# CIS565-Fall-2017/Project3-CUDA-Path-Tracer

Hardware: AMD Instinct MI355X
Metric: Mrays/sec (live paths x bounces) at 800x800 Cornell depth 8 (higher is better)
Workload: dtype f32

## Files before the change

### project3-cuda-path-tracer_amd/csrc/pt_device.hpp

```cpp
#pragma once
#include <hip/hip_runtime.h>
#include <stdint.h>

namespace ptd {

struct f3 { float x, y, z; };

#define PTD __device__ __forceinline__

PTD f3 mk(float x, float y, float z) { f3 r; r.x = x; r.y = y; r.z = z; return r; }
PTD f3 add(f3 a, f3 b) { return mk(a.x + b.x, a.y + b.y, a.z + b.z); }
PTD f3 sub(f3 a, f3 b) { return mk(a.x - b.x, a.y - b.y, a.z - b.z); }
PTD f3 mul(f3 a, f3 b) { return mk(a.x * b.x, a.y * b.y, a.z * b.z); }
PTD f3 scale(f3 a, float s) { return mk(a.x * s, a.y * s, a.z * s); }
PTD f3 neg(f3 a) { return mk(-a.x, -a.y, -a.z); }
PTD float dot(f3 a, f3 b) { return (a.x * b.x + a.y * b.y) + a.z * b.z; }
PTD float length_gated(f3 a);
PTD f3 normalize_gated(f3 a);
PTD float sqrt_gated(float x);
PTD float length(f3 a) { return length_gated(a); }
PTD f3 normalize(f3 a) { return normalize_gated(a); }
PTD f3 normalize_unit(f3 a);
PTD f3 cross(f3 x, f3 y) {
    return mk(x.y * y.z - y.y * x.z, x.z * y.x - y.z * x.x, x.x * y.y - y.x * x.y);
}
PTD f3 cross_axis(f3 x, f3 y) {
    return mk(__builtin_fmaf(x.y, y.z, -(y.y * x.z)), __builtin_fmaf(x.z, y.x, -(y.z * x.x)), __builtin_fmaf(x.x, y.y, -(y.x * x.y)));
}
PTD f3 reflect(f3 I, f3 N) {
    const f3 p = scale(N, dot(N, I));
    return mk(__builtin_fmaf(-2.0f, p.x, I.x), __builtin_fmaf(-2.0f, p.y, I.y), __builtin_fmaf(-2.0f, p.z, I.z));
}

PTD uint32_t utilhash(uint32_t a) {
    a = (a + 0x7ed55d16u) + (a << 12);
    a = (a ^ 0xc761c23cu) ^ (a >> 19);
    a = (a + 0x165667b1u) + (a << 5);
    a = (a + 0xd3a2646cu) ^ (a << 9);
    a = (a + 0xfd7046c5u) + (a << 3);
    a = (a ^ 0xb55a4f09u) ^ (a >> 16);
    return a;
}

PTD uint32_t mod_m31(uint64_t x) {
    uint32_t r = (uint32_t)(x & 0x7fffffffull) + (uint32_t)(x >> 31);
    return r >= 0x7fffffffu ? r - 0x7fffffffu : r;
}

PTD uint32_t lcg_seed(uint32_t s) {
    uint32_t r = mod_m31((uint64_t)s);
    return r == 0u ? 1u : r;
}

PTD uint32_t seeded_engine(int iter, int index, int depth) {
    uint32_t k = (1u << 31) | ((uint32_t)depth << 22) | (uint32_t)iter;
    return lcg_seed(utilhash(k) ^ utilhash((uint32_t)index));
}

PTD float u01(uint32_t &state) {
    state = mod_m31(48271ull * (uint64_t)state);
    return (float)(state - 1u) / 2147483648.0f;
}

PTD void sincos_shared(float x, float &s, float &c) {
    const float TWO_OVER_PI = 0.636619772367581343f;
    const float MAGIC = 12582912.0f;
    const float P1 = 1.57079625129699707031f, P2 = 7.54978941586159635335e-08f, P3 = 5.39030285815811905290e-15f;
    const float S1 = -1.66666671633720398e-01f, S2 = 8.33333190530538559e-03f,
                S3 = -1.98401714442297816e-04f, S4 = 2.72681563728838228e-06f;
    const float C1 = 4.16666530072689056e-02f, C2 = -1.38876168057322502e-03f, C3 = 2.44678121816832572e-05f;
    const float kf = __builtin_fmaf(x, TWO_OVER_PI, MAGIC) - MAGIC;
    const float r1 = __builtin_fmaf(-kf, P1, x);
    const float r = __builtin_fmaf(-kf, P2, r1);
    const float rl = __builtin_fmaf(-kf, P3, __builtin_fmaf(-kf, P2, r1 - r));
    const float z = r * r;
    const float ze = __builtin_fmaf(r, r, -z);
    const float ps = __builtin_fmaf(z, __builtin_fmaf(z, __builtin_fmaf(z, S4, S3), S2), S1);
    const float pc = __builtin_fmaf(z, __builtin_fmaf(z, C3, C2), C1);
    const float hz = 0.5f * z;
    const float w = 1.0f - hz;
    float e = (1.0f - w) - hz;
    e = __builtin_fmaf(-0.5f, ze, e);
    const float u = (r * z) * ps;
    const float sn = r + __builtin_fmaf(rl, w, u);
    const float cs = w + __builtin_fmaf(z * z, pc, __builtin_fmaf(-rl, sn, e));
    const int q = (int)kf & 3;
    float so = (q & 1) ? cs : sn;
    float co = (q & 1) ? sn : cs;
    so = (q & 2) ? -so : so;
    co = ((q + 1) & 2) ? -co : co;
    s = so;
    c = co;
}

PTD f3 hemisphere(f3 normal, uint32_t &rng) {
    const float TWO_PI = 6.2831853071795864769252867665590057683943f;
    const float SQRT_OF_ONE_THIRD = 0.5773502691896257645091487805019574556476f;
    float up = sqrt_gated(u01(rng));
    float over = sqrt_gated(1 - up * up);
    float around = u01(rng) * TWO_PI;
    f3 notN;
    if (__builtin_fabsf(normal.x) < SQRT_OF_ONE_THIRD) notN = mk(1, 0, 0);
    else if (__builtin_fabsf(normal.y) < SQRT_OF_ONE_THIRD) notN = mk(0, 1, 0);
    else notN = mk(0, 0, 1);
    f3 p1 = normalize(cross_axis(normal, notN));
    f3 p2 = normalize_unit(cross(normal, p1));
    float sa, ca;
    sincos_shared(around, sa, ca);
    return add(add(scale(normal, up), scale(p1, ca * over)), scale(p2, sa * over));
}

constexpr int GEOM_WORDS = 40;
constexpr int G_INV = 4, G_FWD = 16, G_INVT = 28;
constexpr int MAT_WORDS = 12;

template <typename P> PTD f3 mv_point(P m, f3 v) {
    f3 r;
    r.x = (m[0] * v.x + m[3] * v.y) + (m[6] * v.z + m[9]);
    r.y = (m[1] * v.x + m[4] * v.y) + (m[7] * v.z + m[10]);
    r.z = (m[2] * v.x + m[5] * v.y) + (m[8] * v.z + m[11]);
    return r;
}
template <typename P> PTD f3 mv_dir(P m, f3 v) {
    f3 r;
    r.x = (m[0] * v.x + m[3] * v.y) + __builtin_fmaf(m[9], 0.0f, m[6] * v.z);
    r.y = (m[1] * v.x + m[4] * v.y) + __builtin_fmaf(m[10], 0.0f, m[7] * v.z);
    r.z = (m[2] * v.x + m[5] * v.y) + __builtin_fmaf(m[11], 0.0f, m[8] * v.z);
    return r;
}

PTD f3 point_on_ray(f3 o, f3 d, float t) { return add(o, scale(normalize_unit(d), (t - .0001f))); }

struct Hit {
    float t;
    int geom;
    int outside;
    f3 aux;
};

PTD f3 face_from_code(int code) {
    const float s = (code & 1) ? 1.0f : -1.0f;
    const int axis = code >> 1;
    return mk(axis == 0 ? s : 0.0f, axis == 1 ? s : 0.0f, axis == 2 ? s : 0.0f);
}

#ifndef PT_FASTDIV
#define PT_FASTDIV 1
#endif
PTD float rcp_refined(float d) {
    float r = __builtin_amdgcn_rcpf(d);
    float e = __builtin_fmaf(-d, r, 1.0f);
    return __builtin_fmaf(e, r, r);
}
PTD float div_by_rcp(float n, float d, float r) {
    float q = n * r;
    float e = __builtin_fmaf(-d, q, n);
    q = __builtin_fmaf(e, r, q);
    e = __builtin_fmaf(-d, q, n);
    return __builtin_fmaf(e, r, q);
}
PTD void sqrt_newton(float x, float &s, float &h) {
    const float y = __builtin_amdgcn_rsqf(x);
    float g = x * y;
    h = 0.5f * y;
    const float r = __builtin_fmaf(-h, g, 0.5f);
    g = __builtin_fmaf(g, r, g);
    h = __builtin_fmaf(h, r, h);
    s = __builtin_fmaf(__builtin_fmaf(-g, g, x), h, g);
}
PTD float sqrt_normal_range(float x) {
    float s, h;
    sqrt_newton(x, s, h);
    return s;
}
PTD float rsqrt_of_root(float x) {
    float s, h;
    sqrt_newton(x, s, h);
    float q = __uint_as_float(__float_as_uint(h + h) + 1u);
    q = __builtin_fmaf(__builtin_fmaf(-s, q, 1.0f), q, q);
    return __builtin_fmaf(__builtin_fmaf(-s, q, 1.0f), q, q);
}
constexpr float NEAR_ONE_LO = 0x1.ffep-1f, NEAR_ONE_HI = 0x1.001p+0f;
PTD float rsqrt_near_one(float x) {
    const float e = x - 1.0f;
    const float w = __builtin_fmaf(e, -0.5f, 0x1.8p-25f);
    const float t = w + (1.0f + 0x1p-10f);
    return t - 0x1p-10f;
}
#ifndef PT_WAVE_ALL_BALLOT
#define PT_WAVE_ALL_BALLOT 1
#endif
PTD bool wave_all(bool p) {
#if PT_WAVE_ALL_BALLOT
    return __builtin_amdgcn_ballot_w64(!p) == 0ull;
#else
    return __all(p);
#endif
}
PTD bool in_range_bits(float x, float lo, float hi) {
    return (__float_as_uint(x) - __float_as_uint(lo)) <= (__float_as_uint(hi) - __float_as_uint(lo));
}
PTD bool all_in_range(float x, float lo, float hi) {
#if PT_FASTDIV
    return wave_all(in_range_bits(x, lo, hi));
#else
    (void)x; (void)lo; (void)hi;
    return false;
#endif
}
// ... 227 lines not shown
```

### project3-cuda-path-tracer_amd/csrc/pt_h_scene.hpp

```cpp
#pragma once

namespace {

int upload_tri_bounds(const pt_scene_desc *d, double Rorigin);

int upload_cull(const pt_scene_desc *d, const pt_camera &cam) {
    const int n = d->num_geoms;
    std::vector<const float *> inv((size_t)std::max(1, n));
    std::vector<char> sph((size_t)std::max(1, n)), skip((size_t)std::max(1, n));
    for (int i = 0; i < n; ++i) {
        inv[(size_t)i] = &d->geoms[i].inverseTransform.m[0][0];
        sph[(size_t)i] = d->geoms[i].type == PT_SPHERE;
        skip[(size_t)i] = d->geoms[i].type == PT_TRIANGLE_MESH;
    }
    const double eye[3] = {(double)cam.position.x, (double)cam.position.y, (double)cam.position.z};
    std::vector<ptcull::Box> boxes;
    std::vector<double> pts(eye, eye + 3);
    for (int t = 0; t < d->num_triangles; ++t) {
        const pt_vec3 *v = &d->triangles[t].v0;
        double m = 0.0;
        for (int k = 0; k < 3; ++k) m = std::max(m, (double)std::fabs(v[k].x) + std::fabs(v[k].y) + std::fabs(v[k].z));
        if (t == 0 || m > pts[3]) { if (pts.size() < 6) pts.resize(6, 0.0); pts[3] = m; pts[4] = 0.0; pts[5] = 0.0; }
    }
    R.scene.rmax = ptcull::make_boxes(inv.data(), reinterpret_cast<const bool *>(sph.data()),
                                      reinterpret_cast<const bool *>(skip.data()), n, pts.data(), (int)(pts.size() / 3), boxes);
    std::vector<float> rec((size_t)std::max(1, n) * CULL_WORDS, 0.0f);
    for (int i = 0; i < n; ++i) {
        float *r = rec.data() + (size_t)i * CULL_WORDS;
        for (int k = 0; k < 3; ++k) ptcull::centre_half(boxes[(size_t)i].lo[k], boxes[(size_t)i].hi[k], r[2 * k], r[2 * k + 1]);
        int ax = 3;
        if (d->geoms[i].type == PT_CUBE && !pt_experiment("PTMI355_NO_AXIS_REJECT"))
            ax = ptcull::reject_row(&d->geoms[i].inverseTransform.m[0][0], &r[7]);
        if (ax == 4 && pt_experiment("PTMI355_NO_ROW_REJECT")) ax = 3;
        const int tw = d->geoms[i].type | (ax << 8);
        memcpy(&r[6], &tw, 4);
        const uint32_t ent = ((uint32_t)d->geoms[i].type << 7) | ((uint32_t)i << 9);
        memcpy(&r[11], &ent, 4);
    }
    if (!R.d_cull) HIPCHK(hipMalloc(&R.d_cull, rec.size() * 4));
    HIPCHK(hipMemcpyAsync(R.d_cull, rec.data(), rec.size() * 4, hipMemcpyHostToDevice, R.stream));
    HIPCHK(hipStreamSynchronize(R.stream));
    R.scene.cull = R.d_cull;
    R.cull_eye_reach = std::fabs(eye[0]) + std::fabs(eye[1]) + std::fabs(eye[2]);
    return upload_tri_bounds(d, (double)R.scene.rmax);
}

void make_tri_bounds(const pt_triangle *tris, int count, double Rorigin, float *out) {
    const double u = 0x1p-24;
    const float pad = ptbvh::spec_pad(reinterpret_cast<const float *>(tris), count);
    const int n4 = (count + 3) & ~3;
    for (int i = 0; i < n4; ++i) {
        float *o = out + (size_t)i * 4;
        if (i >= count) { o[0] = o[1] = o[2] = 0.0f; o[3] = -1.0f; continue; }
        const pt_triangle &t = tris[i];
        const float v0[3] = {t.v0.x, t.v0.y, t.v0.z};
        const float e1[3] = {t.v1.x - t.v0.x, t.v1.y - t.v0.y, t.v1.z - t.v0.z};
        const float e2[3] = {t.v2.x - t.v0.x, t.v2.y - t.v0.y, t.v2.z - t.v0.z};
        double c[3], h2 = 0.0, cinf = 0.0;
        bool fin = true;
        for (int a = 0; a < 3; ++a) {
            const float x1 = v0[a] + e1[a], x2 = v0[a] + e2[a];
            const float lo = std::fmin(v0[a], std::fmin(x1, x2)) - pad, hi = std::fmax(v0[a], std::fmax(x1, x2)) + pad;
            if (!std::isfinite(lo) || !std::isfinite(hi)) fin = false;
            c[a] = 0.5 * ((double)lo + (double)hi);
            const double h = 0.5 * ((double)hi - (double)lo);
            h2 += h * h;
            cinf = std::fmax(cinf, std::fabs(c[a]));
        }
        if (!fin || !std::isfinite(Rorigin)) { o[0] = o[1] = o[2] = 0.0f; o[3] = INFINITY; continue; }
        const double R0 = std::sqrt(h2);
        const double reach = Rorigin + cinf + R0;
        const double delta = 2.0 * 1.7320508075688772 * u * reach;
        const double Rs = (R0 + 4.0 * (delta + 0x1p-19 * reach)) * (1.0 + 0x1p-10);
        for (int a = 0; a < 3; ++a) o[a] = (float)c[a];
        o[3] = ptcull::round_up(Rs * Rs);
        if (!std::isfinite(o[3])) o[3] = INFINITY;
    }
}

void make_tri_records(const float *spheres, int n, _Float16 *records, float frame[4]) {
    double lo[3] = {INFINITY, INFINITY, INFINITY}, hi[3] = {-INFINITY, -INFINITY, -INFINITY};
    for (int i = 0; i < n; ++i) {
        const float *sp = spheres + (size_t)i * 4;
        if (!(sp[3] >= 0.0f) || !std::isfinite(sp[3])) continue;
        for (int a = 0; a < 3; ++a) { lo[a] = std::fmin(lo[a], (double)sp[a]); hi[a] = std::fmax(hi[a], (double)sp[a]); }
    }
    double g[3] = {0.0, 0.0, 0.0}, Rm = 0.0;
    if (lo[0] <= hi[0]) for (int a = 0; a < 3; ++a) g[a] = (double)(float)(0.5 * (lo[a] + hi[a]));
    for (int i = 0; i < n; ++i) {
        const float *sp = spheres + (size_t)i * 4;
        if (!(sp[3] >= 0.0f) || !std::isfinite(sp[3])) continue;
        const double dx = sp[0] - g[0], dy = sp[1] - g[1], dz = sp[2] - g[2];
        Rm = std::fmax(Rm, std::sqrt(dx * dx + dy * dy + dz * dz) + std::sqrt((double)sp[3]));
    }
    Rm = Rm > 0.0 ? Rm * (1.0 + 0x1p-20) : 1.0;
    float ir = (float)(1.0 / Rm);
    if (!(ir > 0.0f) || !std::isfinite(ir)) ir = 1.0f;
    frame[0] = (float)g[0]; frame[1] = (float)g[1]; frame[2] = (float)g[2]; frame[3] = ir;
    auto pair = [](double v, _Float16 &h, _Float16 &l) { h = (_Float16)(float)v; l = (_Float16)(float)(v - (double)(float)h); };
    for (int i = 0; i < n; ++i) {
        const float *sp = spheres + (size_t)i * 4;
        _Float16 *a = records + (size_t)i * 32;
        for (int k = 0; k < 32; ++k) a[k] = (_Float16)0.0f;
        a[29] = (_Float16)1.0f; a[30] = (_Float16)1.0f;
        if (!(sp[3] >= 0.0f)) { a[27] = (_Float16)30000.0f; continue; }
        if (!std::isfinite(sp[3])) { a[27] = (_Float16)-30000.0f; continue; }
        const double c[3] = {(sp[0] - g[0]) * (double)ir, (sp[1] - g[1]) * (double)ir, (sp[2] - g[2]) * (double)ir};
        const double v[9] = {-c[0] * c[0], -c[1] * c[1], -c[2] * c[2], -2.0 * c[0] * c[1], -2.0 * c[0] * c[2], -2.0 * c[1] * c[2], c[0], c[1], c[2]};
        for (int t = 0; t < 9; ++t) { _Float16 h, l; pair(v[t], h, l); a[3 * t] = h; a[3 * t + 1] = h; a[3 * t + 2] = l; }
        _Float16 h, l;
        pair((c[0] * c[0] + c[1] * c[1] + c[2] * c[2]) - (double)sp[3] * (double)ir * (double)ir, h, l);
        a[27] = h; a[28] = l;
    }
}

int upload_tri_bounds(const pt_scene_desc *d, double Rorigin) {
    if (R.mesh_mode != MESH_TILES || d->num_meshes <= 0) return PT_OK;
    size_t recs = 0;
    for (int k = 0; k < d->num_meshes; ++k) recs += (size_t)((d->meshes[k].triangle_count + 63) & ~63);
    std::vector<_Float16> tr(std::max<size_t>(recs, 64) * 32, (_Float16)0.0f);
    std::vector<float> sph;
    size_t off = 0;
    for (int k = 0; k < d->num_meshes; ++k) {
        const pt_mesh &m = d->meshes[k];
        const size_t n64 = (size_t)((m.triangle_count + 63) & ~63);
        sph.assign(n64 * 4, 0.0f);
        make_tri_bounds(d->triangles + m.first_triangle, m.triangle_count, Rorigin, sph.data());
        for (size_t i = (size_t)((m.triangle_count + 3) & ~3); i < n64; ++i) sph[i * 4 + 3] = -1.0f;
        float frame[4];
        make_tri_records(sph.data(), (int)n64, tr.data() + off * 32, frame);
        float *r = R.grec_frames.data() + (size_t)m.geom_index * 4;
        for (int a = 0; a < 4; ++a) r[a] = frame[a];
        off += n64;
    }
    if (!R.d_tri_bound || R.tri_bound_words < tr.size() / 2) {
        if (R.d_tri_bound) { HIPCHK(hipStreamSynchronize(R.stream)); (void)hipFree(R.d_tri_bound); R.d_tri_bound = nullptr; }
        HIPCHK(hipMalloc(&R.d_tri_bound, tr.size() * 2));
        R.tri_bound_words = tr.size() / 2;
    }
    HIPCHK(hipMemcpyAsync(R.d_tri_bound, tr.data(), tr.size() * 2, hipMemcpyHostToDevice, R.stream));
    for (int k = 0; k < d->num_meshes; ++k) {
        const int gi = d->meshes[k].geom_index;
        HIPCHK(hipMemcpyAsync(R.d_geoms + (size_t)gi * ptd::GEOM_WORDS + ptd::G_INV + 7, R.grec_frames.data() + (size_t)gi * 4, 16, hipMemcpyHostToDevice, R.stream));
    }
    HIPCHK(hipStreamSynchronize(R.stream));
    R.scene.tri_rec = R.d_tri_bound;
    return PT_OK;
}

}

namespace one {

static int upload_bvh(const pt_scene_desc *d, std::vector<float> &grec) {
    std::vector<float> nodes, btris, tops;
    std::vector<int32_t> mesh_list;
    float prune = 0.0f;
    int guard = 1;
    R.bvh_info = pt_bvh_info{};
    R.mesh_grids.clear();
    std::vector<int> by_geom((size_t)d->num_meshes);
    for (int k = 0; k < d->num_meshes; ++k) by_geom[(size_t)k] = k;
    std::sort(by_geom.begin(), by_geom.end(), [&](int x, int y) { return d->meshes[x].geom_index < d->meshes[y].geom_index; });
    for (int kk = 0; kk < d->num_meshes; ++kk) {
        const int k = by_geom[(size_t)kk];
        const pt_mesh &m = d->meshes[k];
        if (kk > 0 && d->meshes[by_geom[(size_t)kk - 1]].geom_index == m.geom_index)
            return fail(PT_ERR_INVALID, "pt_init: geom %d owns more than one mesh", m.geom_index);
        ptbvh::Tree tree;
        ptbvh::build(reinterpret_cast<const float *>(d->triangles + m.first_triangle), m.triangle_count, tree, (double)R.scene.rmax);
        const int root = (int)(nodes.size() / BVH_NODE_WORDS);
        const int slot0 = (int)(btris.size() / TRI_WORDS);
        if ((int64_t)slot0 + m.triangle_count >= (1 << ptbvh::LINK_BITS) || tree.num_nodes() >= (1 << ptbvh::LINK_BITS))
            return fail(PT_ERR_INVALID, "pt_init: PT_MESH_BVH holds at most 2^24 triangles (record links are 24 bits)");
        for (int n = 0; n < tree.num_nodes(); ++n) {
            float *w = &tree.nodes[(size_t)n * BVH_NODE_WORDS];
            for (int c = 0; c < 2; ++c) {
                uint32_t link;
                memcpy(&link, &w[6 + c], 4);
                if ((link >> ptbvh::LINK_BITS) & ptbvh::INFO_LEAF) { link += (uint32_t)slot0; memcpy(&w[6 + c], &link, 4); }
            }
        }
        nodes.insert(nodes.end(), tree.nodes.begin(), tree.nodes.end());
        for (int s = 0; s < m.triangle_count; ++s) {
            const int32_t orig = m.first_triangle + tree.order[(size_t)s];
            const pt_triangle &t = d->triangles[orig];
            float r[TRI_WORDS] = {t.v0.x, t.v0.y, t.v0.z,
                                  t.v1.x - t.v0.x, t.v1.y - t.v0.y, t.v1.z - t.v0.z,
                                  t.v2.x - t.v0.x, t.v2.y - t.v0.y, t.v2.z - t.v0.z, 0.0f, 0.0f, 0.0f};
            memcpy(&r[9], &orig, 4);
// ... 108 lines not shown
```

### project3-cuda-path-tracer_amd/csrc/pt_k_bounce.hpp

```cpp
#pragma once

namespace {

enum { MODE_FUSED = 0, MODE_ISECT = 1, MODE_CACHE0 = 2 };

template <typename T>
__device__ __forceinline__ T karg_field(size_t offset) {
    const __attribute__((address_space(4))) char *kp = (const __attribute__((address_space(4))) char *)__builtin_amdgcn_kernarg_segment_ptr();
    asm volatile("" : "+s"(kp));
    return *(const __attribute__((address_space(4))) T *)(kp + offset);
}
template <typename T>
__device__ __forceinline__ T karg_struct(size_t offset) {
    static_assert(sizeof(T) % 4 == 0, "whole dwords");
    const __attribute__((address_space(4))) char *kp = (const __attribute__((address_space(4))) char *)__builtin_amdgcn_kernarg_segment_ptr();
    asm volatile("" : "+s"(kp));
    uint32_t w[sizeof(T) / 4];
#pragma unroll
    for (size_t k = 0; k < sizeof(T) / 4; ++k) w[k] = *(const __attribute__((address_space(4))) uint32_t *)(kp + offset + 4 * k);
    T t;
    __builtin_memcpy(&t, w, sizeof(T));
    return t;
}
__device__ __forceinline__ Pool karg_pool(size_t offset) {
    return Pool{karg_field<float *>(offset + offsetof(Pool, base)), karg_field<uint32_t>(offset + offsetof(Pool, cap))};
}

struct TileCtx {
    bool kargs = false;
    bool kmisc = false;
    bool epi_direct = false;
    SceneAcc acc;
    float *tri_lds;
    int lane, iter0;
    uint32_t stamp;
};

struct TileRegs {
    bool have, active;
    uint32_t i, src, tile, pid, smp;
    int pixel;
    f3 col;
    MeshBest mb;
};

template <bool GEN, bool RESOLVE = false>
__device__ __forceinline__ void tile_load(const BounceArgs &a, const TileCtx &c, const Pool &in, int depth,
                                          uint32_t tile, uint32_t i, uint32_t src, bool have, bool active,
                                          TileRegs &tr, f3 &ro, f3 &rd) {
    constexpr bool gen_rays = GEN;
    tr.have = have; tr.i = i; tr.src = src; tr.tile = tile;
    tr.pid = DEAD_PID; tr.smp = 0; tr.pixel = 0;
    tr.col = ptd::mk(1.0f, 1.0f, 1.0f);
    tr.mb.t = FLT_MAX; tr.mb.geom = -1; tr.mb.tri = -1;
    ro = ptd::mk(0, 0, 0); rd = ptd::mk(0, 0, 1);
    if (active) {
        if (gen_rays) {
            tr.pid = i;
        } else {
            const SlotPtr p = (c.kargs ? karg_pool(offsetof(BounceArgs, in)) : in).slot(src);
            tr.pid = ppid(p);
            ro = ptd::mk(pf(p, 0), pf(p, 1), pf(p, 2));
            rd = ptd::mk(pf(p, 3), pf(p, 4), pf(p, 5));
            tr.col = ptd::mk(pf(p, 6), pf(p, 7), pf(p, 8));
            if (tr.pid == DEAD_PID) active = false;
        }
    }
    bool pending = false;
    if (RESOLVE && active) { pending = (tr.pid & PENDING_DIR) != 0u; tr.pid &= ~PENDING_DIR; }
    if (active) {
        if (c.kmisc) {
            const TileMap map = karg_struct<TileMap>(offsetof(BounceArgs, map));
            tr.smp = sample_of(map, tr.pid);
            tr.pixel = local_to_pixel(map, (int)(tr.pid - tr.smp * (uint32_t)map.tile_pixels));
            if (gen_rays) camera_ray(karg_struct<pt_camera>(offsetof(BounceArgs, cam)), karg_struct<Lens>(offsetof(BounceArgs, lens)),
                                     karg_field<int>(offsetof(BounceArgs, trace_depth)), c.iter0 + (int)tr.smp, tr.pixel, map.W, ro, rd);
        } else {
            tr.smp = sample_of(a.map, tr.pid);
            tr.pixel = local_to_pixel(a.map, (int)(tr.pid - tr.smp * (uint32_t)a.map.tile_pixels));
            if (gen_rays) camera_ray(a.cam, a.lens, a.trace_depth, c.iter0 + (int)tr.smp, tr.pixel, a.map.W, ro, rd);
        }
    }
    if (RESOLVE && pending) {
        uint32_t rng = ptd::seeded_engine(c.iter0 + (int)tr.smp, tr.pixel, depth - 1);
        rd = ptd::hemisphere(rd, rng);
    }
    tr.active = active;
}

__device__ __forceinline__ bool mesh_root_candidate(const int4 *bvh_meshes, int bvh_nmesh, const float *geoms, const float *bvh_nodes, f3 ro, f3 rd) {
    bool cand = false;
#pragma unroll 1
    for (int k = 0; k < bvh_nmesh; ++k) {
        const __attribute__((address_space(4))) int *mrec =
            (const __attribute__((address_space(4))) int *)(unsigned long long)(bvh_meshes + k);
        cfloat *grid = as_const(geoms) + (size_t)mrec[0] * ptd::GEOM_WORDS + ptd::G_INV;
        const __attribute__((address_space(4))) uint32_t *b =
            (const __attribute__((address_space(4))) uint32_t *)(unsigned long long)(bvh_nodes + (size_t)mrec[1] * BVH_NODE_WORDS);
        const BvhRay br = bvh_ray(ro, rd, ptd::mk(grid[0], grid[1], grid[2]), ptd::mk(grid[3], grid[4], grid[5]));
        float tn, tf;
        bvh_slab(br, b[0], b[1], b[2], tn, tf);
        cand |= tn <= tf;
        bvh_slab(br, b[3], b[4], b[5], tn, tf);
        cand |= tn <= tf;
    }
    return cand;
}
__device__ __forceinline__ bool mesh_root_candidate(const SceneDev &sc, f3 ro, f3 rd) {
    return mesh_root_candidate(sc.bvh_meshes, sc.bvh_nmesh, sc.geoms, sc.bvh_nodes, ro, rd);
}

template <bool COMPACT, int MESH = MESH_NONE, bool SORT = false, bool DEFER = false>
__device__ __forceinline__ void tile_shade(const BounceArgs &a, const TileCtx &c, const Pool &in, const Pool &out, int depth,
                                           const TileRegs &tr, f3 ro, f3 rd, float t, f3 nrm, int mat, int outside,
                                           uint32_t n, uint32_t dst_base, uint32_t &packed, uint32_t &traced,
                                           uint32_t key_stride = 0) {
    const int lane = c.lane;
    bool alive = false, deferred = false;
    ptd::PathState ps;
    ps.o = ro; ps.d = rd; ps.c = tr.col;
    if (tr.active) {
        const bool defer = DEFER && (c.kargs ? karg_field<int>(offsetof(BounceArgs, defer_dir)) : a.defer_dir) != 0;
        alive = ptd::shade_scatter(ps, t, nrm, mat, outside, c.acc.mats, c.iter0 + (int)tr.smp, tr.pixel, depth,
                                   depth == a.trace_depth - 1, defer, &deferred);
        if (!alive) {
            if (c.epi_direct) {
                if (!(ps.c.x == 0.0f && ps.c.y == 0.0f && ps.c.z == 0.0f)) {
                    float *img = karg_field<float *>(offsetof(BounceArgs, epi_image)) + 3 * (size_t)tr.pixel;
                    const float r = img[0] + ps.c.x, g = img[1] + ps.c.y, b = img[2] + ps.c.z;
                    img[0] = r; img[1] = g; img[2] = b;
                    float *host = karg_field<float *>(offsetof(BounceArgs, epi_host));
                    if (host) { host += 3 * (size_t)tr.pixel; host[0] = r; host[1] = g; host[2] = b; }
                }
            } else {
                put_final((c.kargs || c.kmisc) ? karg_field<float *>(offsetof(BounceArgs, fin)) : a.fin, tr.pid, ps.c, c.stamp);
            }
        }
    }
    const uint64_t bal = ballot64(alive);
    const uint64_t act = ballot64(tr.active);
    traced += (uint32_t)__popcll((unsigned long long)act);
    uint32_t dst = tr.i;
    if (COMPACT && SORT) {
        for_each_key(alive, (uint32_t)mat, [&](uint32_t k, uint64_t m) {
            const uint32_t have = (uint32_t)__builtin_amdgcn_readlane((int)packed, (int)k);
            if (alive && (uint32_t)mat == k) dst = k * key_stride + dst_base + have + rank_below(m);
            if ((uint32_t)lane == k) packed += (uint32_t)__popcll((unsigned long long)m);
        });
    } else if (COMPACT) {
        dst = dst_base + packed + rank_below(bal);
        packed += (uint32_t)__popcll((unsigned long long)bal);
    }
    if (alive) {
        const SlotPtr p = (c.kargs ? karg_pool(offsetof(BounceArgs, out)) : out).slot(dst);
        pf(p, 0) = ps.o.x; pf(p, 1) = ps.o.y; pf(p, 2) = ps.o.z;
        pf(p, 3) = ps.d.x; pf(p, 4) = ps.d.y; pf(p, 5) = ps.d.z;
        pf(p, 6) = ps.c.x; pf(p, 7) = ps.c.y; pf(p, 8) = ps.c.z;
        ppid(p) = deferred ? (tr.pid | PENDING_DIR) : tr.pid;
        if (MESH == MESH_PRE) {
            constexpr size_t SC = offsetof(BounceArgs, scene);
            const bool reach = c.kargs
                ? mesh_root_candidate(karg_field<const int4 *>(SC + offsetof(SceneDev, bvh_meshes)), karg_field<int>(SC + offsetof(SceneDev, bvh_nmesh)),
                                      karg_field<const float *>(SC + offsetof(SceneDev, geoms)), karg_field<const float *>(SC + offsetof(SceneDev, bvh_nodes)), ps.o, ps.d)
                : mesh_root_candidate(a.scene, ps.o, ps.d);
            if (reach)
                atomicOr(&(c.kargs ? karg_field<unsigned long long *>(offsetof(BounceArgs, mesh_flags_out)) : a.mesh_flags_out)[dst >> 6], 1ull << (dst & 63u));
        }
    } else if (!COMPACT && tr.have && tr.i < n) {
        out.pid(dst) = DEAD_PID;
    }
}

template <bool COMPACT, int MESH, bool SORT = false, bool DEFER = false>
__device__ __forceinline__ void tile_finish(const BounceArgs &a, const TileCtx &c, const WaveQ &q, int par, const Pool &in,
                                            const Pool &out, int depth, const TileRegs &tr, uint32_t n, uint32_t dst_base,
                                            uint32_t &packed, uint32_t &traced, uint32_t key_stride = 0) {
    const float *ry = q.rays(par) + c.lane;
    const f3 ro = ptd::mk(ry[0], ry[64], ry[128]);
    const f3 rd = ptd::mk(ry[192], ry[256], ry[320]);
    float t = -1.0f; f3 nrm = ptd::mk(0, 0, 0); int mat = 0, outside = 1;
    if (tr.active) tile_result(q, par, c.acc, a.scene.tris, tr.mb, t, nrm, mat, outside);
    tile_shade<COMPACT, MESH, SORT, DEFER>(a, c, in, out, depth, tr, ro, rd, t, nrm, mat, outside, n, dst_base, packed, traced, key_stride);
}

struct WgSpans {
    uint32_t p1, p2, p3, total;
    uint32_t b0, b1, b2, b3;
};

template <int MODE, bool COMPACT, int MESH, bool GEN, bool SORT = false, bool DEFER = false, bool RESOLVE = false>
__device__ __forceinline__ void run_tiles(const BounceArgs &a, const TileCtx &c, WaveQ &q, const Pool &in, const Pool &out,
                                          int depth, uint32_t first_tile, uint32_t count, uint32_t tiles,
                                          uint32_t n, bool packed_in, uint32_t span_in, uint32_t &cur, uint32_t dst_base,
                                          bool own_span, const WgSpans &ws, uint32_t &packed, uint32_t &traced,
                                          uint32_t key_stride = 0, bool aligned = false) {
    const int lane = c.lane;
    bool pending = false;
    TileRegs prev{};
    uint32_t prev_ticket = 0;
    int par = 0;
    const bool masked = MODE == MODE_FUSED && GEN && a.cull0 != nullptr;
    uint32_t mtile = masked ? first_tile % a.cull0_tiles : 0u;
    for (uint32_t r = 0; r < count; ++r) {
        const uint32_t tile = first_tile + r;
        if (!own_span && tile >= tiles) break;
        rotate_priority(r + (uint32_t)depth, PT_MIN_WAVES + 1);
        unsigned long long gmask = 0;
        if (masked) {
            gmask = ((const __attribute__((address_space(4))) unsigned long long *)(unsigned long long)a.cull0)[mtile];
            if (++mtile == a.cull0_tiles) mtile = 0;
        }
        bool have, active;
        uint32_t i, src;
        if (own_span) {
            const uint32_t L = tile * TILE + lane;
            have = true; active = L < ws.total;
            uint32_t off = L, b = ws.b0;
            if (L >= ws.p1) { off = L - ws.p1; b = ws.b1; }
            if (L >= ws.p2) { off = L - ws.p2; b = ws.b2; }
            if (L >= ws.p3) { off = L - ws.p3; b = ws.b3; }
            src = b + off; i = src;
        } else if (aligned) {
            have = tile < tiles;
            active = false; i = 0; src = 0;
            if (have) {
                const uint32_t *tb = a.dir_in.tbase();
                while (tile >= tb[cur + 1]) ++cur;
                const uint32_t t64 = (tile - tb[cur]) * TILE + (uint32_t)lane;
                active = t64 < a.dir_in.count()[cur];
                src = cur * span_in + t64;
                i = a.dir_in.base()[cur] + t64;
            }
        } else {
            have = tile < tiles;
            i = tile * TILE + lane;
            active = have && i < n;
            src = i;
// ... 304 lines not shown
```

### project3-cuda-path-tracer_amd/csrc/pt_k_intersect.hpp

```cpp
#pragma once

namespace {

template <int MESH>
__device__ __forceinline__ void cull_scene(const SceneDev &sc, const SceneAcc &acc, WaveQ &q, int par, float *tri_lds,
                                           bool active, f3 ro, f3 rd, MeshBest &mb, const float4 *pre_hit,
                                           bool masked = false, unsigned long long gmask = 0) {
    const int lane = threadIdx.x & 63;
    {
        float *ry = q.rays(par) + lane;
        ry[0] = ro.x; ry[64] = ro.y; ry[128] = ro.z; ry[192] = rd.x; ry[256] = rd.y; ry[320] = rd.z;
        q.best(par)[lane] = ~0ull;
    }
    mb.t = FLT_MAX; mb.geom = -1; mb.tri = -1;
    if (MESH == MESH_PRE && pre_hit) {
        const float4 m = *pre_hit;
        mb.t = m.x; mb.geom = __float_as_int(m.y); mb.tri = __float_as_int(m.z);
    }
    const CullRay cr = cull_ray(ro, rd, sc.rmax);
    const uint64_t m_act = ballot64(active), m_wild = ballot64(cr.wild);
    CULL_STAT(0, 1); CULL_STAT(5, __popcll((unsigned long long)ballot64(active && cr.wild))); CULL_STAT(6, __popcll((unsigned long long)ballot64(active)));
    const uint32_t tag = (uint32_t)lane | ((uint32_t)par << 6);
    cfloat *cc = as_const(sc.cull);
    cfloat *const cc_end = cc + sc.ngeoms * CULL_WORDS;
    for (; cc != cc_end; cc += CULL_WORDS) {
        float cb[12];
#pragma unroll
        for (int k = 0; k < 12; ++k) cb[k] = cc[k];
        uint32_t ent = (uint32_t)__builtin_amdgcn_readfirstlane((int)__float_as_uint(cb[11]));
        asm volatile("" : "+s"(ent));
        const int g = (int)(ent >> 9);
        if (masked && !((gmask >> (g & 63)) & 1ull)) continue;
        const int tw = __float_as_int(cb[6]);
        const int type = tw & 0xff;
        if (MESH != MESH_NONE && type == PT_TRIANGLE_MESH) {
            if (MESH == MESH_PRE) continue;
            cfloat *rec = as_const(sc.geoms) + g * ptd::GEOM_WORDS;
            float best = FLT_MAX;
            int best_i = -1;
            if (MESH == MESH_BVH) {
                const int root = __float_as_int(rec[2]);
                const int count = __float_as_int(rec[3]);
                if (active && count > 0)
                    bvh_walk(sc.bvh_nodes + (size_t)root * BVH_NODE_WORDS, sc.bvh_tris, rec + ptd::G_INV, sc.bvh_prune,
                             sc.bvh_guard, ro, rd, best, best_i, cr.wild);
            } else {
                const int first = __float_as_int(rec[2]);
                const int count = __float_as_int(rec[3]);
                const int boff = __float_as_int(rec[ptd::G_INV + 6]);
                mesh_sweep(sc, q, par, tri_lds, first, count, boff, rec[ptd::G_INV + 7], rec[ptd::G_INV + 8], rec[ptd::G_INV + 9], rec[ptd::G_INV + 10],
                           ro, rd, m_act, m_wild, best, best_i);
            }
            if (active && best_i >= 0) {
                f3 p = ptd::add(ro, ptd::scale(rd, best));
                const float t = ptd::length(ptd::sub(ro, p));
                if (t > 0.0f && mb.t > t) { mb.t = t; mb.geom = g; mb.tri = best_i; }
            }
            continue;
        }
        const uint64_t m = m_act & cull_candidates(cr, m_wild, ro, rd, cb[0], cb[1], cb[2], cb[3], cb[4], cb[5], tw, cb[7], cb[8], cb[9], cb[10]);
        if (m) {
            if (lane_of(m)) {
                const uint32_t s = (q.total + rank_below(m)) & (Q_SLOTS - 1);
                q.ring()[s] = tag | ent;
            }
            q.total += (uint32_t)__popcll((unsigned long long)m);
            CULL_STAT(1, __popcll((unsigned long long)m));
            __builtin_amdgcn_fence(__ATOMIC_ACQ_REL, "wavefront");
            if (q.total - q.head >= 64) {
                cand_pass(q, acc, q.head, 64);
                q.head += 64;
            }
        }
    }
}

__device__ __forceinline__ void drain_to(WaveQ &q, const SceneAcc &acc, uint32_t ticket) {
    while ((int32_t)(ticket - q.head) > 0) {
        const uint32_t cnt = min(64u, q.total - q.head);
        cand_pass(q, acc, q.head, cnt);
        q.head += cnt;
    }
}

__device__ __forceinline__ void tile_result(const WaveQ &q, int par, const SceneAcc &acc, const float *__restrict__ tris,
                                            const MeshBest &mb, float &t, f3 &n, int &mat, int &outside) {
    const int lane = threadIdx.x & 63;
    const unsigned long long key = q.best(par)[lane];
    t = -1.0f; n = ptd::mk(0, 0, 0); mat = 0; outside = 1;
    int geom = -1;
    uint32_t info = 0;
    if (key != ~0ull) {
        const uint32_t lo = (uint32_t)key;
        t = __uint_as_float((uint32_t)(key >> 32)); geom = (int)(lo >> 4); outside = (int)(lo & 1u);
        info = acc.ginfo[geom];
        if ((info >> 28) == (uint32_t)PT_CUBE) {
            const float *f = acc.grec + (size_t)geom * GREC_WORDS + GREC_FACE + 3 * ((lo >> 1) & 7u);
            n = ptd::mk(f[0], f[1], f[2]);
        } else {
            const float *w = q.win(par) + lane;
            n = ptd::mk(w[0], w[64], w[128]);
        }
    }
    if (mb.geom >= 0 && (geom < 0 || t > mb.t || (t == mb.t && mb.geom < geom))) {
        const float *tv = tris + (size_t)mb.tri * TRI_WORDS;
        t = mb.t; geom = mb.geom; outside = 1;
        n = ptd::normalize(ptd::cross(ptd::mk(tv[3], tv[4], tv[5]), ptd::mk(tv[6], tv[7], tv[8])));
        info = acc.ginfo[geom];
    }
    if (geom >= 0) mat = (int)(info & 0x0fffffffu);
}


struct LdsCarve { float *scene, *pw, *tri; };
__device__ __forceinline__ LdsCarve carve_lds(float *lds_raw, const SceneDev &sc, bool slds) {
    LdsCarve c;
    c.scene = lds_raw + LDS_CTL_WORDS;
    float *after = c.scene + (slds ? scene_lds_words(sc.nmats, sc.ngeoms) : 0);
    c.pw = after + (threadIdx.x >> 6) * PW_WORDS;
    c.tri = after + WAVES * PW_WORDS + (threadIdx.x >> 6) * TRQ_WORDS;
    return c;
}

template <int MESH, bool SLDS, bool GEN = false>
__global__ __launch_bounds__(BLOCK, PT_ISECT_WAVES) void k_intersect(Pool in, Isect out, SceneDev sc,
                                                                    const uint32_t *n_ptr, uint32_t n_fixed,
                                                                    RangeDir dir_in, const uint32_t *nprev_ptr,
                                                                    Control *ctl, const unsigned long long *cull0,
                                                                    uint32_t cull0_tiles, RayGen gen) {
    extern __shared__ __attribute__((aligned(16))) float lds_raw[];
    const LdsCarve lc = carve_lds(lds_raw, sc, SLDS);
    const SceneAcc acc = stage_scene<SLDS>(lc.scene, sc);
    WaveQ q{lc.pw, 0, 0};
    const int lane = threadIdx.x & 63;
    const uint32_t W = gridDim.x * WAVES;
    const uint32_t wid = run_id();
    const uint32_t n = n_ptr ? *n_ptr : n_fixed;
    const uint32_t tiles = (n + TILE - 1) / TILE;
    const uint32_t R = range_tiles(n, W);
    const bool packed = dir_in.mem && nprev_ptr;
    const uint32_t span = packed ? *dir_in.span() : 0;
    uint32_t cur = 0;
    if (packed && wid * R < tiles) cur = find_range(dir_in.base(), dir_in.nr, wid * R * TILE);
    auto finish = [&](uint32_t i, int par, const MeshBest &mb) {
        if (i < n) {
            float t; f3 nrm; int mat, outside;
            tile_result(q, par, acc, sc.tris, mb, t, nrm, mat, outside);
            out.plane(0)[i] = t; out.plane(1)[i] = nrm.x; out.plane(2)[i] = nrm.y; out.plane(3)[i] = nrm.z;
            out.mat()[i] = mat | (outside ? 0 : (int)0x80000000u);
        }
    };
    bool pending = false;
    uint32_t prev_i = 0, prev_ticket = 0;
    MeshBest prev_mb{FLT_MAX, -1, -1};
    int par = 0;
    const bool masked = cull0 != nullptr;
    uint32_t mtile = masked ? (wid * R) % cull0_tiles : 0u;
    for (uint32_t r = 0; r < R; ++r) {
        const uint32_t tile = wid * R + r;
        if (tile >= tiles) break;
        rotate_priority(r, PT_ISECT_WAVES + 1);
        const bool have = tile < tiles;
        const uint32_t i = tile * TILE + lane;
        bool active = have && i < n;
        uint32_t src = i;
        if (packed && have) src = resolve_src(dir_in, span, cur, i, active, ctl);
        unsigned long long gmask = 0;
        if (masked) {
            gmask = ((const __attribute__((address_space(4))) unsigned long long *)(unsigned long long)cull0)[mtile];
            if (++mtile == cull0_tiles) mtile = 0;
        }
        f3 ro = ptd::mk(0, 0, 0), rd = ptd::mk(0, 0, 1);
        if (GEN && active) {
            const uint32_t smp = sample_of(gen.map, i);
            const int pixel = local_to_pixel(gen.map, (int)(i - smp * (uint32_t)gen.map.tile_pixels));
            camera_ray(gen.cam, gen.lens, gen.trace_depth, gen.iter0 + (int)smp, pixel, gen.map.W, ro, rd);
        } else if (!GEN && active) {
            const SlotPtr p = in.slot(src);
            if (ppid(p) == DEAD_PID) active = false;
            ro = ptd::mk(pf(p, 0), pf(p, 1), pf(p, 2));
            rd = ptd::mk(pf(p, 3), pf(p, 4), pf(p, 5));
        }
        MeshBest mb;
        cull_scene<MESH>(sc, acc, q, par, lc.tri, active, ro, rd, mb, nullptr, masked, gmask);
        const uint32_t ticket = q.total;
        if (pending) { drain_to(q, acc, prev_ticket); finish(prev_i, par ^ 1, prev_mb); }
        prev_i = have ? i : 0xffffffffu; prev_mb = mb; prev_ticket = ticket; pending = true; par ^= 1;
    }
    if (pending) { drain_to(q, acc, prev_ticket); finish(prev_i, par ^ 1, prev_mb); }
}

__global__ __launch_bounds__(BLOCK) void k_cull0_mask(SceneDev sc, pt_camera cam, TileMap map, int trace_depth,
                                                     unsigned long long *mask, uint32_t ntiles) {
    const int lane = threadIdx.x & 63;
    const uint32_t tile = blockIdx.x * WAVES + (threadIdx.x >> 6);
    if (tile >= ntiles) return;
    const Lens pinhole{0, 0.0f, 0.0f};
    f3 ro, rd;
    camera_ray(cam, pinhole, trace_depth, 0, local_to_pixel(map, (int)(tile * TILE + lane)), map.W, ro, rd);
    const CullRay cr = cull_ray(ro, rd, sc.rmax);
    const uint64_t m_wild = ballot64(cr.wild);
    unsigned long long bits = 0;
    for (int g = 0; g < sc.ngeoms; ++g) {
        float cb[11];
        cfloat *cn = as_const(sc.cull) + g * CULL_WORDS;
#pragma unroll
        for (int k = 0; k < 11; ++k) cb[k] = cn[k];
        const bool mesh = (__float_as_int(cb[6]) & 0xff) == PT_TRIANGLE_MESH;
        if (mesh || cull_candidates(cr, m_wild, ro, rd, cb[0], cb[1], cb[2], cb[3], cb[4], cb[5], __float_as_int(cb[6]), cb[7],
                                    cb[8], cb[9], cb[10]) != 0)
            bits |= 1ull << (g & 63);
    }
    if (lane == 0) mask[tile] = bits;
}


template <int MESH, bool SLDS>
__global__ __launch_bounds__(BLOCK, PT_MIN_WAVES) void k_cache_first(Isect cache, SceneDev sc, pt_camera cam,
                                                                      TileMap map) {
    extern __shared__ __attribute__((aligned(16))) float lds_raw[];
    const LdsCarve lc = carve_lds(lds_raw, sc, SLDS);
    const SceneAcc acc = stage_scene<SLDS>(lc.scene, sc);
    WaveQ q{lc.pw, 0, 0};
    const uint32_t n = (uint32_t)map.tile_pixels;
    const uint32_t tiles = (n + BLOCK - 1) / BLOCK;
    for (uint32_t tile = blockIdx.x; tile < tiles; tile += gridDim.x) {
// ... 18 lines not shown
```

### project3-cuda-path-tracer_amd/csrc/pt_k_scene.hpp

```cpp
#pragma once

namespace {

constexpr int LDS_CTL_WORDS = 32;
constexpr int GREC_WORDS = 52;
constexpr int GREC_FACE = 24;
constexpr int Q_SLOTS = 128;
constexpr int PW_RING = 0;
constexpr int PW_BEST = PW_RING + Q_SLOTS;
constexpr int PW_WIN = PW_BEST + 2 * 64 * 2;
constexpr int PW_RAYS = PW_WIN + 2 * 64 * 3;
constexpr int PW_WORDS = PW_RAYS + 2 * 6 * 64;
constexpr int CULL_WORDS = 12;

__host__ __device__ constexpr int scene_lds_words(int nmats, int ngeoms) {
    return ((nmats * ptd::MAT_WORDS + 3) & ~3) + ((ngeoms + 3) & ~3) + ngeoms * GREC_WORDS;
}

struct SceneAcc {
    const float *mats;
    const uint32_t *ginfo;
    const float *grec;
};

template <bool SLDS>
__device__ __forceinline__ SceneAcc stage_scene(float *lds_scene, const SceneDev &sc) {
    SceneAcc acc;
    if (!SLDS) {
        acc.mats = sc.mats; acc.ginfo = sc.ginfo; acc.grec = sc.grec;
        return acc;
    }
    const int mw = sc.nmats * ptd::MAT_WORDS;
    float *mats = lds_scene;
    uint32_t *ginfo = reinterpret_cast<uint32_t *>(lds_scene + ((mw + 3) & ~3));
    float *grec = lds_scene + ((mw + 3) & ~3) + ((sc.ngeoms + 3) & ~3);
    for (int k = threadIdx.x; k < mw; k += BLOCK) mats[k] = sc.mats[k];
    for (int k = threadIdx.x; k < sc.ngeoms; k += BLOCK) ginfo[k] = sc.ginfo[k];
    {
        const float4 *src = reinterpret_cast<const float4 *>(sc.grec);
        float4 *dst = reinterpret_cast<float4 *>(grec);
        for (int k = threadIdx.x; k < sc.ngeoms * (GREC_WORDS / 4); k += BLOCK) dst[k] = src[k];
    }
    __syncthreads();
    acc.mats = mats; acc.ginfo = ginfo; acc.grec = grec;
    return acc;
}

__global__ __launch_bounds__(BLOCK) void k_face_normals(float *grec, const uint32_t *ginfo, int ngeoms) {
    const int k = (int)(blockIdx.x * BLOCK + threadIdx.x);
    if (k >= ngeoms * 8) return;
    const int g = k >> 3, code = k & 7;
    float *r = grec + (size_t)g * GREC_WORDS;
    if ((ginfo[g] >> 28) != (uint32_t)PT_CUBE) return;
    const f3 n = ptd::normalize(ptd::mv_dir(r + 12, ptd::face_from_code(code)));
    float *f = r + GREC_FACE + 3 * code;
    f[0] = n.x; f[1] = n.y; f[2] = n.z;
}

typedef const __attribute__((address_space(4))) float cfloat;
__device__ __forceinline__ cfloat *as_const(const float *p) {
    return (cfloat *)(unsigned long long)p;
}

struct CullRay {
    float ix, iy, iz, nx, ny, nz;
    bool wild;
};
__device__ __forceinline__ CullRay cull_ray(f3 ro, f3 rd, float rmax) {
    CullRay c;
    const float os = (__builtin_fabsf(ro.x) + __builtin_fabsf(ro.y)) + __builtin_fabsf(ro.z);
    const float ds = (__builtin_fabsf(rd.x) + __builtin_fabsf(rd.y)) + __builtin_fabsf(rd.z);
    c.wild = !(os <= rmax) || !(ds >= 9.5367431640625e-07f && ds <= 1048576.0f);
    c.ix = __builtin_amdgcn_fmed3f(__builtin_amdgcn_rcpf(rd.x), -0x1p100f, 0x1p100f);
    c.iy = __builtin_amdgcn_fmed3f(__builtin_amdgcn_rcpf(rd.y), -0x1p100f, 0x1p100f);
    c.iz = __builtin_amdgcn_fmed3f(__builtin_amdgcn_rcpf(rd.z), -0x1p100f, 0x1p100f);
    c.nx = -ro.x * c.ix; c.ny = -ro.y * c.iy; c.nz = -ro.z * c.iz;
    return c;
}
__device__ __forceinline__ bool cull_box(const CullRay &c, float cx, float hx, float cy, float hy, float cz, float hz) {
    const float tmx = __builtin_fmaf(cx, c.ix, c.nx), tmy = __builtin_fmaf(cy, c.iy, c.ny), tmz = __builtin_fmaf(cz, c.iz, c.nz);
    const float tnx = __builtin_fmaf(-hx, __builtin_fabsf(c.ix), tmx), tfx = __builtin_fmaf(hx, __builtin_fabsf(c.ix), tmx);
    const float tny = __builtin_fmaf(-hy, __builtin_fabsf(c.iy), tmy), tfy = __builtin_fmaf(hy, __builtin_fabsf(c.iy), tmy);
    const float tnz = __builtin_fmaf(-hz, __builtin_fabsf(c.iz), tmz), tfz = __builtin_fmaf(hz, __builtin_fabsf(c.iz), tmz);
    const float tn = __builtin_fmaxf(__builtin_fmaxf(tnx, tny), __builtin_fmaxf(tnz, 0.0f));
    const float tf = __builtin_fminf(__builtin_fminf(tfx, tfy), tfz);
    return !(tn > tf);
}

#ifndef PT_CULL_ROW
#define PT_CULL_ROW 1
#endif
__device__ __forceinline__ uint64_t cull_candidates(const CullRay &cr, uint64_t m_wild, f3 ro, f3 rd, float cx, float hx,
                                                    float cy, float hy, float cz, float hz, int tw, float m0, float m1,
                                                    float m2, float m3) {
    uint64_t keep = ballot64(cull_box(cr, cx, hx, cy, hy, cz, hz));
#if PT_CULL_ROW == 2
    {
        (void)tw;
        const float qk = (m0 * ro.x + m1 * ro.y) + (m2 * ro.z + m3);
        const float vk = (m0 * rd.x + m1 * rd.y) + m2 * rd.z;
        keep &= ~(ballot64(__builtin_fabsf(qk) > 0.5f) & ballot64(qk * vk > 0.0f));
    }
#elif PT_CULL_ROW == 1
    {
        float qk, vk;
        if (tw & 0x400) {
            qk = (m0 * ro.x + m1 * ro.y) + (m2 * ro.z + m3);
            vk = (m0 * rd.x + m1 * rd.y) + m2 * rd.z;
        } else {
            qk = __builtin_fmaf(m2, ro.z, __builtin_fmaf(m1, ro.y, m0 * ro.x)) + m3;
            vk = __builtin_fmaf(m2, rd.z, __builtin_fmaf(m1, rd.y, m0 * rd.x));
        }
        keep &= ~(ballot64(__builtin_fabsf(qk) > 0.5f) & ballot64(qk * vk > 0.0f));
    }
#else
    const int rmode = (tw >> 8) & 7;
    if (rmode != 3) {
        float qk, vk;
        if (rmode == 4) {
            qk = (m0 * ro.x + m1 * ro.y) + (m2 * ro.z + m3);
            vk = (m0 * rd.x + m1 * rd.y) + m2 * rd.z;
        } else if (rmode == 0) {
            qk = m0 * ro.x + m3; vk = m0 * rd.x;
        } else if (rmode == 1) {
            qk = m1 * ro.y + m3; vk = m1 * rd.y;
        } else {
            qk = m2 * ro.z + m3; vk = m2 * rd.z;
        }
        keep &= ~(ballot64(__builtin_fabsf(qk) > 0.5f) & ballot64(qk * vk > 0.0f));
    }
#endif
    return keep | m_wild;
}

struct WaveQ {
    float *pw;
    uint32_t head, total;
    __device__ __forceinline__ uint32_t *ring() const { return reinterpret_cast<uint32_t *>(pw + PW_RING); }
    __device__ __forceinline__ unsigned long long *best(int par) const {
        return reinterpret_cast<unsigned long long *>(pw + PW_BEST) + par * 64;
    }
    __device__ __forceinline__ float *win(int par) const { return pw + PW_WIN + par * 3 * 64; }
    __device__ __forceinline__ float *rays(int par) const { return pw + PW_RAYS + par * 6 * 64; }
};

#ifdef PT_CULL_STATS
__device__ unsigned long long g_cull_stats[8];
#define CULL_STAT(k, v) do { if ((threadIdx.x & 63) == 0) atomicAdd(&g_cull_stats[k], (unsigned long long)(v)); } while (0)
#else
#define CULL_STAT(k, v) do {} while (0)
#endif

__device__ __forceinline__ void cand_pass1(const WaveQ &q, const SceneAcc &acc, uint32_t head, uint32_t count);
__device__ __forceinline__ void cand_pass(const WaveQ &q, const SceneAcc &acc, uint32_t head, uint32_t count) {
    cand_pass1(q, acc, head, count);
#ifdef PT_DBG_PASS2
    cand_pass1(q, acc, head, count);
#endif
}
__device__ __forceinline__ void cand_pass1(const WaveQ &q, const SceneAcc &acc, uint32_t head, uint32_t count) {
    const int lane = threadIdx.x & 63;
    CULL_STAT(2, 1); CULL_STAT(3, count);
    if ((uint32_t)lane < count) {
        const uint32_t e = q.ring()[(head + (uint32_t)lane) & (Q_SLOTS - 1)];
        const int origin = (int)(e & 63u), par = (int)((e >> 6) & 1u), type = (int)((e >> 7) & 3u);
        const uint32_t g = e >> 9;
        const float *ry = q.rays(par) + origin;
        const f3 ro = ptd::mk(ry[0], ry[64], ry[128]);
        const f3 rd = ptd::mk(ry[192], ry[256], ry[320]);
        const float4 *rec4 = reinterpret_cast<const float4 *>(acc.grec + (size_t)g * GREC_WORDS);
        float m[12];
        {
            const float4 a = rec4[0], b = rec4[1], c = rec4[2];
            m[0] = a.x; m[1] = a.y; m[2] = a.z; m[3] = a.w; m[4] = b.x; m[5] = b.y; m[6] = b.z; m[7] = b.w;
            m[8] = c.x; m[9] = c.y; m[10] = c.z; m[11] = c.w;
        }
        f3 qo, v;
        float x;
        ptd::object_ray(m, ro, rd, qo, v, x);
        const f3 qd = ptd::normalize_with(v, x, ptd::norm_fast_ok(x));
        float t_obj = 0.0f;
        int code = 7, outside = 1;
        bool hit = false;
        if (type == PT_CUBE) {
            hit = ptd::cube_slabs(qo, qd, ptd::cube_fast_ok(qo, v, x), t_obj, code, outside);
        } else {
            hit = ptd::sphere_roots(qo, qd, t_obj, outside);
        }
        CULL_STAT(4, __popcll((unsigned long long)ballot64(hit)));
        if (hit) {
            {
                const float4 a = rec4[3], b = rec4[4], c = rec4[5];
                m[0] = a.x; m[1] = a.y; m[2] = a.z; m[3] = a.w; m[4] = b.x; m[5] = b.y; m[6] = b.z; m[7] = b.w;
                m[8] = c.x; m[9] = c.y; m[10] = c.z; m[11] = c.w;
            }
            f3 obj_p;
            const float t = ptd::world_distance(m, ro, qo, qd, t_obj, obj_p);
            if (t > 0.0f) {
                const unsigned long long key = ((unsigned long long)__float_as_uint(t) << 32) | (g << 4) |
                                               ((uint32_t)code << 1) | (uint32_t)(outside & 1);
                unsigned long long *bk = q.best(par) + origin;
                __hip_atomic_fetch_min(bk, key, __ATOMIC_RELAXED, __HIP_MEMORY_SCOPE_WAVEFRONT);
                if (type != PT_CUBE) {
                    const float4 a = rec4[6], b = rec4[7], c = rec4[8];
                    m[0] = a.x; m[1] = a.y; m[2] = a.z; m[3] = a.w; m[4] = b.x; m[5] = b.y; m[6] = b.z; m[7] = b.w;
                    m[8] = c.x; m[9] = c.y; m[10] = c.z; m[11] = c.w;
                    f3 n = ptd::normalize(ptd::mv_dir(m, obj_p));
                    if (!outside) n = ptd::neg(n);
                    __builtin_amdgcn_fence(__ATOMIC_ACQ_REL, "wavefront");
                    if (*bk == key) { float *w = q.win(par) + origin; w[0] = n.x; w[64] = n.y; w[128] = n.z; }
                }
            }
        }
    }
    __builtin_amdgcn_fence(__ATOMIC_ACQ_REL, "wavefront");
}

}
```

Measured before the change: 54080.

## Batch cull candidates per geometry chunk and hoist wave-uniform RNG key hash

The culling loop now gathers a per-lane bitmask of candidate geometries over chunks of 32 and then enqueues them in a separate pass. The old code did a ballot, ring write, fence and drain check for every geometry. The geometry type moves out of the queue entry and is looked up from ginfo in cand_pass, so the cull record stores only the geometry id. Separately, the RNG key hash is computed once per wave when all lanes share the same sample index, with a fallback when they differ. Risks include an extra LDS read of ginfo per candidate and a change in enqueue order, which may alter queue batching.

```diff
diff --git a/project3-cuda-path-tracer_amd/csrc/pt_device.hpp b/project3-cuda-path-tracer_amd/csrc/pt_device.hpp
--- a/project3-cuda-path-tracer_amd/csrc/pt_device.hpp
+++ b/project3-cuda-path-tracer_amd/csrc/pt_device.hpp
@@ -52,9 +52,14 @@
     return r == 0u ? 1u : r;
 }
 
+PTD uint32_t engine_key_hash(int iter, int depth) {
+    return utilhash((1u << 31) | ((uint32_t)depth << 22) | (uint32_t)iter);
+}
+PTD uint32_t seeded_engine_kh(uint32_t key_hash, int index) {
+    return lcg_seed(key_hash ^ utilhash((uint32_t)index));
+}
 PTD uint32_t seeded_engine(int iter, int index, int depth) {
-    uint32_t k = (1u << 31) | ((uint32_t)depth << 22) | (uint32_t)iter;
-    return lcg_seed(utilhash(k) ^ utilhash((uint32_t)index));
+    return seeded_engine_kh(engine_key_hash(iter, depth), index);
 }
 
 PTD float u01(uint32_t &state) {
diff --git a/project3-cuda-path-tracer_amd/csrc/pt_h_scene.hpp b/project3-cuda-path-tracer_amd/csrc/pt_h_scene.hpp
--- a/project3-cuda-path-tracer_amd/csrc/pt_h_scene.hpp
+++ b/project3-cuda-path-tracer_amd/csrc/pt_h_scene.hpp
@@ -34,8 +34,8 @@
         if (ax == 4 && pt_experiment("PTMI355_NO_ROW_REJECT")) ax = 3;
         const int tw = d->geoms[i].type | (ax << 8);
         memcpy(&r[6], &tw, 4);
-        const uint32_t ent = ((uint32_t)d->geoms[i].type << 7) | ((uint32_t)i << 9);
-        memcpy(&r[11], &ent, 4);
+        const uint32_t gid = (uint32_t)i;
+        memcpy(&r[11], &gid, 4);
     }
     if (!R.d_cull) HIPCHK(hipMalloc(&R.d_cull, rec.size() * 4));
     HIPCHK(hipMemcpyAsync(R.d_cull, rec.data(), rec.size() * 4, hipMemcpyHostToDevice, R.stream));
diff --git a/project3-cuda-path-tracer_amd/csrc/pt_k_bounce.hpp b/project3-cuda-path-tracer_amd/csrc/pt_k_bounce.hpp
--- a/project3-cuda-path-tracer_amd/csrc/pt_k_bounce.hpp
+++ b/project3-cuda-path-tracer_amd/csrc/pt_k_bounce.hpp
@@ -82,7 +82,10 @@
         }
     }
     if (RESOLVE && pending) {
-        uint32_t rng = ptd::seeded_engine(c.iter0 + (int)tr.smp, tr.pixel, depth - 1);
+        const uint32_t smp0 = (uint32_t)__builtin_amdgcn_readfirstlane((int)tr.smp);
+        uint32_t kh = ptd::engine_key_hash(c.iter0 + (int)smp0, depth - 1);
+        if (ballot64(tr.smp != smp0) != 0ull) kh = ptd::engine_key_hash(c.iter0 + (int)tr.smp, depth - 1);
+        uint32_t rng = ptd::seeded_engine_kh(kh, tr.pixel);
         rd = ptd::hemisphere(rd, rng);
     }
     tr.active = active;
diff --git a/project3-cuda-path-tracer_amd/csrc/pt_k_intersect.hpp b/project3-cuda-path-tracer_amd/csrc/pt_k_intersect.hpp
--- a/project3-cuda-path-tracer_amd/csrc/pt_k_intersect.hpp
+++ b/project3-cuda-path-tracer_amd/csrc/pt_k_intersect.hpp
@@ -1,6 +1,24 @@
 #pragma once
 
 namespace {
+
+constexpr int CAND_CHUNK = 32;
+__device__ __forceinline__ void queue_candidates(WaveQ &q, const SceneAcc &acc, uint32_t tagb, uint32_t cand) {
+    asm volatile("" : "+v"(tagb));
+    for (uint64_t m = ballot64(cand != 0u); m; m = ballot64(cand != 0u)) {
+        if (lane_of(m)) {
+            const uint32_t s = __builtin_amdgcn_mbcnt_hi((uint32_t)(m >> 32), __builtin_amdgcn_mbcnt_lo((uint32_t)m, q.total));
+            q.ring()[s & (Q_SLOTS - 1)] = tagb + ((uint32_t)__builtin_ctz(cand) << 9);
+        }
+        cand &= cand - 1u;
+        q.total += (uint32_t)__popcll((unsigned long long)m);
+        __builtin_amdgcn_fence(__ATOMIC_ACQ_REL, "wavefront");
+        if (q.total - q.head >= 64) {
+            cand_pass(q, acc, q.head, 64);
+            q.head += 64;
+        }
+    }
+}
 
 template <int MESH>
 __device__ __forceinline__ void cull_scene(const SceneDev &sc, const SceneAcc &acc, WaveQ &q, int par, float *tri_lds,
@@ -23,55 +41,52 @@
     const uint32_t tag = (uint32_t)lane | ((uint32_t)par << 6);
     cfloat *cc = as_const(sc.cull);
     cfloat *const cc_end = cc + sc.ngeoms * CULL_WORDS;
-    for (; cc != cc_end; cc += CULL_WORDS) {
-        float cb[12];
+    for (uint32_t base = 0; cc != cc_end; base += CAND_CHUNK) {
+        cfloat *const chunk_end = (cc_end - cc > CAND_CHUNK * CULL_WORDS) ? cc + CAND_CHUNK * CULL_WORDS : cc_end;
+        uint32_t cand = 0;
+        for (; cc != chunk_end; cc += CULL_WORDS) {
+            float cb[12];
 #pragma unroll
-        for (int k = 0; k < 12; ++k) cb[k] = cc[k];
-        uint32_t ent = (uint32_t)__builtin_amdgcn_readfirstlane((int)__float_as_uint(cb[11]));
-        asm volatile("" : "+s"(ent));
-        const int g = (int)(ent >> 9);
-        if (masked && !((gmask >> (g & 63)) & 1ull)) continue;
-        const int tw = __float_as_int(cb[6]);
-        const int type = tw & 0xff;
-        if (MESH != MESH_NONE && type == PT_TRIANGLE_MESH) {
-            if (MESH == MESH_PRE) continue;
-            cfloat *rec = as_const(sc.geoms) + g * ptd::GEOM_WORDS;
-            float best = FLT_MAX;
-            int best_i = -1;
-            if (MESH == MESH_BVH) {
-                const int root = __float_as_int(rec[2]);
-                const int count = __float_as_int(rec[3]);
-                if (active && count > 0)
-                    bvh_walk(sc.bvh_nodes + (size_t)root * BVH_NODE_WORDS, sc.bvh_tris, rec + ptd::G_INV, sc.bvh_prune,
-                             sc.bvh_guard, ro, rd, best, best_i, cr.wild);
-            } else {
-                const int first = __float_as_int(rec[2]);
-                const int count = __float_as_int(rec[3]);
-                const int boff = __float_as_int(rec[ptd::G_INV + 6]);
-                mesh_sweep(sc, q, par, tri_lds, first, count, boff, rec[ptd::G_INV + 7], rec[ptd::G_INV + 8], rec[ptd::G_INV + 9], rec[ptd::G_INV + 10],
-                           ro, rd, m_act, m_wild, best, best_i);
+            for (int k = 0; k < 12; ++k) cb[k] = cc[k];
+            uint32_t gid = (uint32_t)__builtin_amdgcn_readfirstlane((int)__float_as_uint(cb[11]));
+            asm volatile("" : "+s"(gid));
+            const int g = (int)gid;
+            if (masked && !((gmask >> (g & 63)) & 1ull)) continue;
+            const int tw = __float_as_int(cb[6]);
+            const int type = tw & 0xff;
+            if (MESH != MESH_NONE && type == PT_TRIANGLE_MESH) {
+                if (MESH == MESH_PRE) continue;
+                cfloat *rec = as_const(sc.geoms) + g * ptd::GEOM_WORDS;
+                float best = FLT_MAX;
+                int best_i = -1;
+                if (MESH == MESH_BVH) {
+                    const int root = __float_as_int(rec[2]);
+                    const int count = __float_as_int(rec[3]);
+                    if (active && count > 0)
+                        bvh_walk(sc.bvh_nodes + (size_t)root * BVH_NODE_WORDS, sc.bvh_tris, rec + ptd::G_INV, sc.bvh_prune,
+                                 sc.bvh_guard, ro, rd, best, best_i, cr.wild);
+                } else {
+                    const int first = __float_as_int(rec[2]);
+                    const int count = __float_as_int(rec[3]);
+                    const int boff = __float_as_int(rec[ptd::G_INV + 6]);
+                    mesh_sweep(sc, q, par, tri_lds, first, count, boff, rec[ptd::G_INV + 7], rec[ptd::G_INV + 8], rec[ptd::G_INV + 9], rec[ptd::G_INV + 10],
+                               ro, rd, m_act, m_wild, best, best_i);
+                }
+                if (active && best_i >= 0) {
+                    f3 p = ptd::add(ro, ptd::scale(rd, best));
+                    const float t = ptd::length(ptd::sub(ro, p));
+                    if (t > 0.0f && mb.t > t) { mb.t = t; mb.geom = g; mb.tri = best_i; }
+                }
+                continue;
             }
-            if (active && best_i >= 0) {
-                f3 p = ptd::add(ro, ptd::scale(rd, best));
-                const float t = ptd::length(ptd::sub(ro, p));
-                if (t > 0.0f && mb.t > t) { mb.t = t; mb.geom = g; mb.tri = best_i; }
+            const uint64_t m = m_act & cull_candidates(cr, m_wild, ro, rd, cb[0], cb[1], cb[2], cb[3], cb[4], cb[5], tw, cb[7], cb[8], cb[9], cb[10]);
+            CULL_STAT(1, __popcll((unsigned long long)m));
+            if (lane_of(m)) {
+                asm volatile("");
+                cand |= 1u << (g & (CAND_CHUNK - 1));
             }
-            continue;
-        }
-        const uint64_t m = m_act & cull_candidates(cr, m_wild, ro, rd, cb[0], cb[1], cb[2], cb[3], cb[4], cb[5], tw, cb[7], cb[8], cb[9], cb[10]);
-        if (m) {
-            if (lane_of(m)) {
-                const uint32_t s = (q.total + rank_below(m)) & (Q_SLOTS - 1);
-                q.ring()[s] = tag | ent;
-            }
-            q.total += (uint32_t)__popcll((unsigned long long)m);
-            CULL_STAT(1, __popcll((unsigned long long)m));
-            __builtin_amdgcn_fence(__ATOMIC_ACQ_REL, "wavefront");
-            if (q.total - q.head >= 64) {
-                cand_pass(q, acc, q.head, 64);
-                q.head += 64;
-            }
-        }
+        }
+        queue_candidates(q, acc, tag + (base << 9), cand);
     }
 }
 
diff --git a/project3-cuda-path-tracer_amd/csrc/pt_k_scene.hpp b/project3-cuda-path-tracer_amd/csrc/pt_k_scene.hpp
--- a/project3-cuda-path-tracer_amd/csrc/pt_k_scene.hpp
+++ b/project3-cuda-path-tracer_amd/csrc/pt_k_scene.hpp
@@ -163,8 +163,9 @@
     CULL_STAT(2, 1); CULL_STAT(3, count);
     if ((uint32_t)lane < count) {
         const uint32_t e = q.ring()[(head + (uint32_t)lane) & (Q_SLOTS - 1)];
-        const int origin = (int)(e & 63u), par = (int)((e >> 6) & 1u), type = (int)((e >> 7) & 3u);
+        const int origin = (int)(e & 63u), par = (int)((e >> 6) & 1u);
         const uint32_t g = e >> 9;
+        const int type = (int)(acc.ginfo[g] >> 28);
         const float *ry = q.rays(par) + origin;
         const f3 ro = ptd::mk(ry[0], ry[64], ry[128]);
         const f3 rd = ptd::mk(ry[192], ry[256], ry[320]);
```

After: 53290 (median of 2 runs). 1.5% lower.
